# daniestevez/ldpc-toolbox

Hardware: AMD Instinct MI355X
Metric: codewords/s + info-bits/s, DVB-S2 n=64800 r=1/2 min-sum 50 iters (higher is better)
Workload: dtype f32

## Files before the change

ldpc_toolbox_amd/csrc/c_api.cpp:

```cpp
#include "../../include/ldpc_toolbox.h"

#include <algorithm>
#include <cerrno>
#include <cstdio>
#include <cstdlib>
#include <cstring>
#include <fstream>
#include <memory>
#include <sstream>
#include <string>
#include <vector>

#include "codes.h"
#include "demodulator.h"
#include "device_bch.h"
#include "device_decoder.h"
#include "device_encoder.h"
#include "device_nr_rm.h"
#include "device_nr_tb.h"
#include "encoder.h"
#include "implementation.h"
#include "simulator.h"
#include "sparse.h"

// ... 815 lines not shown
    *value = d.last_lanes();
  else if (k == "last_pooled")
    *value = static_cast<int64_t>(d.last_pooled());
  else if (k == "last_group")
    *value = static_cast<int64_t>(d.last_group());
  else if (k == "preferred_group")
    *value = static_cast<int64_t>(d.preferred_group(size_t(1) << 20));
  else if (k == "row_records")
    *value = d.row_records();
  else if (k == "record_flag_bits")
    *value = d.record_flag_bits();
  else if (k == "last_vn_records")
    *value = d.last_vn_records();
  else if (k == "last_vn_bundles")
    *value = d.last_vn_bundles();
  else if (k == "vn_bundle_saved_permille")
    *value = d.vn_bundle_saved_permille();
  else if (k == "last_vn_chains")
    *value = d.last_vn_chains();
  else if (k == "vn_chain_saved_permille")
    *value = d.vn_chain_saved_permille();
  else if (k == "flags8")
    *value = d.flags8();
  else if (k == "last_record_flag_bytes")
    *value = d.last_record_flag_bytes();
  else if (k == "call_edges")
    *value = d.call_edges();
  else if (k == "last_call_edges")
    *value = d.last_call_edges();
  else if (k == "minsum_correction")
    *value = static_cast<int64_t>(d.implementation().correction);
  else if (k == "minsum_correction_int")
    *value = d.implementation().correction_int;
  else if (k == "last_persist" || k == "experiments")
    *value = 0;
  else
    return -1;
  return 0;
}

int32_t ldpc_toolbox_decoder_set(void *decoder, const char *key, int64_t value) {
  auto *h = static_cast<DecoderHandle *>(decoder);
  if (!h || !h->dec || !key) return -1;
  const std::string k = key;
  if (k == "group_size" && value >= 0)
    h->dec->set_group_size(static_cast<size_t>(value));
// ... 574 lines not shown
```

ldpc_toolbox_amd/csrc/device_decoder.h:

```cpp
#pragma once
#include <hip/hip_runtime_api.h>

#include <algorithm>
#include <atomic>
#include <cstddef>
#include <cstdint>
#include <memory>
#include <string>
#include <vector>

#include "hip_owned.h"
#include "implementation.h"
#include "sparse.h"

namespace ldpc {

struct GroupCall;

struct KernelStat {
  uint64_t launches = 0;
  double total_ms = 0.0;
};

enum KernelKind { kKernelCheck = 0, kKernelVar = 1, kKernelLayer = 2, kKernelOther = 3, kKernelKinds = 4 };
// ... 5 lines not shown
  ~DeviceDecoder();

  size_t n() const { return n_; }
  size_t m() const { return m_; }
  size_t edges() const { return e_; }
  size_t input_len() const { return input_len_; }
  const Implementation &implementation() const { return impl_; }
  int device() const { return device_; }
  uint32_t max_check_degree() const { return max_row_weight_; }
  uint32_t max_variable_degree() const { return max_col_weight_; }
  size_t layers() const { return level_ptr_.empty() ? 0 : level_ptr_.size() - 1; }
  uint32_t last_lanes() const { return last_lanes_; }
  uint64_t last_pooled() const { return last_pooled_; }
  size_t last_group() const { return last_group_; }
  uint32_t row_records() const { return (rec_ready_ && records_wanted() && opt_lfree_ && !opt_staged_minsum_) ? rec_w_ : 0; }
  uint32_t record_flag_bits() const { return row_records() ? rec_flag_bits_ : 0; }
  uint32_t last_vn_records() const { return last_vn_records_.load(std::memory_order_relaxed) ? 1 : 0; }
  uint32_t flags8() const { return opt_flags8_ ? 1 : 0; }
  uint32_t last_record_flag_bytes() const { return last_record_flag_bytes_.load(std::memory_order_relaxed); }
  uint32_t last_vn_bundles() const { return last_vn_bundles_.load(std::memory_order_relaxed) ? 1 : 0; }
  uint32_t vn_bundle_saved_permille() const { return last_vn_bundle_saved_.load(std::memory_order_relaxed); }
  uint32_t last_vn_chains() const { return last_vn_chains_.load(std::memory_order_relaxed) ? 1 : 0; }
  uint32_t vn_chain_saved_permille() const { return last_vn_chain_saved_.load(std::memory_order_relaxed); }
  uint32_t call_edges() const { return opt_call_edges_ ? 1 : 0; }
  uint32_t last_call_edges() const { return last_call_edges_.load(std::memory_order_relaxed); }
  static constexpr uint32_t kCallEdgeIngest = 1;
  static constexpr uint32_t kCallEdgeClose = 2;
  static constexpr uint32_t kCallEdgeEmit = 4;
  static constexpr uint32_t kCallEdgeCheckpoint = 8;

  void set_group_size(size_t g) { group_pref_ = g; }
  size_t group_size() const { return group_pref_; }
  void set_min_group(size_t g) { min_group_ = g; }
  size_t preferred_group(size_t batch) const { return pick_group(batch); }
  bool set_option(const std::string &key, int64_t value);
  void set_profiling(bool on);
  KernelStat kernel_stat(int kind);
  void reset_kernel_stats();

  int decode_device(const void *llrs, bool llrs_f64, size_t batch, uint32_t max_iterations,
                    uint8_t *bits, size_t out_len, int32_t *iterations, void *posterior,
                    hipStream_t stream);

  int decode_host(const void *llrs, bool llrs_f64, size_t batch, uint32_t max_iterations,
                  uint8_t *bits, size_t out_len, int32_t *iterations, void *posterior);

// ... 57 lines not shown
  std::string error_;

  uint32_t n_keep_ = 0, n_free_ = 0;
  uint32_t post_rows_keep_ = 0;
  bool opt_rec_long_ = false;
  bool opt_rec_quiet_ = true;
  bool opt_vn_event_ = true;
  bool opt_vn_records_ = false;
  bool opt_flags8_ = false;
  bool opt_vn_bundles_ = false;
  static constexpr uint32_t kVnBundleW = kStreamBlock / 64;
  uint32_t vn_bundle_saved_[kVnBundleW + 1] = {};
  std::atomic<bool> last_vn_bundles_{false};
  std::atomic<uint32_t> last_vn_bundle_saved_{0};
  bool opt_vn_chains_ = false;
  uint32_t opt_vn_chain_len_ = 8;
  static constexpr uint32_t kVnChainLens[3] = {4, 8, 16};
  struct VnChainAt {
    uint32_t rs_at = 0, var_at = 0, ptr_at = 0, n_blocks = 0;
    uint32_t saved = 0, saved_alone = 0;
  } vn_chain_at_[3];
  std::atomic<bool> last_vn_chains_{false};
  std::atomic<uint32_t> last_vn_chain_saved_{0};
  bool opt_call_edges_ = true;
  std::atomic<uint32_t> last_call_edges_{0};
  std::atomic<uint32_t> last_record_flag_bytes_{0};
  std::atomic<bool> last_vn_records_{false};
  uint32_t rec_w_ = 0;
  uint32_t rec_flag_bits_ = 0;
  bool rec_ready_ = false, rec_prefers_ = false;
  uint32_t opt_records_ = 1;
  bool records_wanted() const { return opt_records_ >= 2 || (opt_records_ == 1 && rec_prefers_); }
  uint32_t opt_rec_run_ = 8;
  bool opt_compact_ = true;
  uint32_t opt_compact_first_ = 0, opt_compact_every_ = 0;
  uint32_t opt_serial_levels_ = 512;
  uint32_t opt_cn_reg_ = 1;
  uint32_t opt_hl_reg_ = 1;
  bool opt_lane_threads_ = true, opt_throttle_ = false;
  uint32_t opt_lead_ = 0;
  bool opt_lane_pace_ = true;
  bool opt_hl_records_ = true;
  std::vector<uint32_t> level_maxdeg_;
  std::vector<uint32_t> level_rec_ptr_;
  bool lfree_ready_ = false, opt_lfree_ = true;
  std::vector<uint32_t> level_ptr_;
// ... 56 lines not shown
```

ldpc_toolbox_amd/csrc/device_decoder.hip:

```cpp
#define LDPC_GROUP_KERNELS_TU 1
#include "codes.h"
#include "device_decoder_internal.h"

namespace ldpc {

static bool is_dvbs2_half_rate_normal(const SparseMatrix::Csr &g) {
  if (g.n_cols != 64800 || g.n_rows != 32400) return false;
  SparseMatrix ref;
  if (!codes::dvbs2("R1_2", &ref)) return false;
  const SparseMatrix::Csr r = ref.csr();
  if (r.n_edges != g.n_edges || r.row_ptr != g.row_ptr) return false;
  std::vector<uint32_t> a, b;
  for (uint32_t row = 0; row < g.n_rows; row++) {
    a.assign(g.edge_col.begin() + g.row_ptr[row], g.edge_col.begin() + g.row_ptr[row + 1]);
    b.assign(r.edge_col.begin() + r.row_ptr[row], r.edge_col.begin() + r.row_ptr[row + 1]);
    std::sort(a.begin(), a.end());
    std::sort(b.begin(), b.end());
    if (a != b) return false;
  }
  return true;
}

bool DeviceDecoder::fail(const std::string &msg, hipError_t e) {
  static std::mutex m;
// ... 71 lines not shown
    *dst = upload(v, &e);
    return e == hipSuccess;
  };
  g.edge_col.resize(g.edge_col.size() + kTablePad, 0);
  bool ok = up(g.row_ptr, &d->d_row_ptr_) && up(g.edge_col, &d->d_edge_col_) && up(g.col_ptr, &d->d_col_ptr_) &&
            up(g.col_edge, &d->d_col_edge_);
  const bool flooding_minsum = impl.schedule == Schedule::Flooding && impl.rule == Rule::Minsum && !impl.i8;
  if (ok && flooding_minsum) {
    const LfreeTables lf = build_lfree_tables(g);
    if (lf.ready) {
      d->n_keep_ = lf.n_keep;
      d->n_free_ = lf.n_free;
      d->post_rows_keep_ = lf.post_rows_keep;
      ok = up(lf.aux, &d->d_edge_aux_) && up(lf.keep_var, &d->d_keep_var_) && up(lf.keep_ptr, &d->d_keep_ptr_) &&
           up(lf.keep_edge, &d->d_keep_edge_) && up(lf.free_var, &d->d_free_var_) && up(lf.free_ptr, &d->d_free_ptr_) &&
           up(lf.free_edge, &d->d_free_edge_);
      d->lfree_ready_ = ok;
    }
    const RowRecordTables rr = d->lfree_ready_ ? build_row_record_tables(g, lf, impl.f64) : RowRecordTables();
    if (rr.ready) {
      d->rec_prefers_ = rr.rec_prefers;
      d->rec_w_ = rr.rec_w;
      d->rec_flag_bits_ = rr.flag_bits;
      ok = up(rr.keep_pos, &d->d_keep_pos_) && up(rr.peer, &d->d_edge_peer_) && up(rr.free_rs, &d->d_free_rs_);
      d->rec_ready_ = ok;
      const KeepRsTable kr = (ok && rr.flag_bits == 16) ? build_keep_rs(g, lf) : KeepRsTable();
      if (kr.ready) {
        const VnBundleTables vb = build_vn_bundles(lf.n_keep, lf.keep_ptr, lf.keep_var, kr.rs, kVnBundleW);
        std::vector<uint32_t> words = kr.rs;
        auto append = [&](const std::vector<uint32_t> &v) {
          const uint32_t at = static_cast<uint32_t>(words.size());
          words.insert(words.end(), v.begin(), v.end());
          return at;
        };
        d->bundle_rs_at_ = append(vb.keep_rs);
        d->bundle_var_at_ = append(vb.list_var);
        d->bundle_ptr_at_ = append(vb.list_ptr);
        for (uint32_t c = 0; c < 3; c++) {
          const VnChainTables vc = build_vn_chains(lf.n_keep, lf.keep_ptr, lf.keep_var, kr.rs, kVnBundleW, kVnChainLens[c]);
          VnChainAt &at = d->vn_chain_at_[c];
          at.rs_at = append(vc.keep_rs);
          at.var_at = append(vc.list_var);
          at.ptr_at = append(vc.list_ptr);
          at.n_blocks = vc.n_blocks;
          at.saved = vc.fetches ? static_cast<uint32_t>((vc.fetches - vc.issued) * 1000 / vc.fetches) : 0;
          at.saved_alone = vc.fetches ? static_cast<uint32_t>(vc.carried * 1000 / vc.fetches) : 0;
        }
        ok = up(words, &d->d_keep_rs_);
        for (uint32_t w = 2; w <= kVnBundleW; w++) {
          uint64_t fetches = 0, distinct = 0;
          count_vn_bundle_fetches(lf.n_keep, vb.list_ptr, vb.keep_rs, w, &fetches, &distinct);
          d->vn_bundle_saved_[w] = fetches ? static_cast<uint32_t>((fetches - distinct) * 1000 / fetches) : 0;
        }
      }
      d->opt_vn_records_ = kr.ready && ok && !impl.f64 && impl.correction == Correction::None && is_dvbs2_half_rate_normal(g);
      d->opt_flags8_ = d->opt_vn_records_;
      d->opt_vn_bundles_ = d->opt_vn_records_ && d->bundle_rs_at_ != 0;
      d->opt_vn_chains_ = d->opt_vn_bundles_ && d->vn_chain_at_[0].rs_at != 0;
    }
  }
  if (ok && flooding_minsum && !impl.f64) {
    SlicedTables st = build_sliced_tables(g);
    if (st.ready) {
      d->lat_ = std::make_unique<LatencyPath>();
      d->lat_->tables = std::move(st);
    }
  }
  if (ok && impl.schedule == Schedule::Flooding && impl.rule == Rule::Tanh && !impl.i8 && d->max_row_weight_ <= kLevelRecShort) {
    LevelTables all;
    all.level_ptr = {0u, g.n_rows};
    all.rows.resize(g.n_rows);
    for (uint32_t r = 0; r < g.n_rows; r++) all.rows[r] = r;
    all.maxdeg = {d->max_row_weight_};
    ok = up(build_level_recs(all, g.row_ptr, g.edge_col).words, &d->d_row_recs_);
  }
  LevelTables lt;
  if (ok && impl.schedule == Schedule::Layered) {
    lt = build_levels(g.row_ptr, g.edge_col, g.n_rows, g.n_cols);
    d->level_ptr_ = lt.level_ptr;
    d->level_maxdeg_ = lt.maxdeg;
    const LevelRecs lr = build_level_recs(lt, g.row_ptr, g.edge_col);
// ... 41 lines not shown
bool DeviceDecoder::set_option(const std::string &key, int64_t value) {
  if (value < 0) return false;
  const uint32_t v = static_cast<uint32_t>(value);
  if (key == "waves")
    opt_waves_ = v;
  else if (key == "vec")
    opt_vec_ = v;
  else if (key == "tile")
    opt_tile_ = v;
  else if (key == "lfree")
    opt_lfree_ = v != 0;
  else if (key == "records")
    opt_records_ = v != 0 ? (v >= 2 ? 2 : 1) : 0;
  else if (key == "rec_run")
    opt_rec_run_ = std::max<uint32_t>(v, 1);
  else if (key == "rec_quiet")
    opt_rec_quiet_ = v != 0;
  else if (key == "vn_event")
    opt_vn_event_ = v != 0;
  else if (key == "vn_records")
    opt_vn_records_ = v != 0;
  else if (key == "flags8")
    opt_flags8_ = v != 0;
  else if (key == "vn_bundles")
    opt_vn_bundles_ = v != 0;
  else if (key == "vn_chains")
    opt_vn_chains_ = v != 0;
  else if (key == "vn_chain_len") {
    if (v != kVnChainLens[0] && v != kVnChainLens[1] && v != kVnChainLens[2]) return false;
    opt_vn_chain_len_ = v;
  }
  else if (key == "rec_long")
    opt_rec_long_ = v != 0;
  else if (key == "call_edges")
    opt_call_edges_ = v != 0;
  else if (key == "compact")
    opt_compact_ = v != 0;
  else if (key == "staged_minsum")
    opt_staged_minsum_ = v != 0;
  else if (key == "hl_reg")
    opt_hl_reg_ = v;
  else if (key == "cn_reg")
    opt_cn_reg_ = v;
  else if (key == "hl_records")
    opt_hl_records_ = v != 0;
  else if (key == "lane_threads")
// ... 819 lines not shown
```

ldpc_toolbox_amd/csrc/graph_tables.h:

```cpp
#pragma once
#include <algorithm>
#include <cstdint>
#include <vector>

#include "record_flags8.h"
#include "slice_tasks.h"
#include "sparse.h"

namespace ldpc {

namespace dev {
enum : uint32_t { kAuxNone = 0xFFFFFFFFu, kAuxWriter = 0x80000000u, kAuxSingle = 0x7FFFFFFEu, kAuxMask = 0x7FFFFFFFu };
enum : uint32_t { kPeerKeep = 0x80000000u, kPeerPosMask = 0x7FFFFFFFu, kPeerWriter = 0x40000000u, kPeerRowMask = 0xFFFFFFu,
                  kPeerSingle = 0xFFFFFFu };
enum : uint32_t { kNoLane = 0xFFFFFFFFu };
}

constexpr uint32_t kTablePad = 16;

struct LfreeTables {
  bool ready = false;
  std::vector<uint32_t> aux, keep_var, keep_ptr{0}, keep_edge, free_var, free_ptr{0}, free_edge;
  uint32_t n_keep = 0, n_free = 0;
  uint32_t post_rows_keep = 0;
};
// ... 62 lines not shown
  }
  size_t far_peers = 0, near_peers = 0;
  for (size_t i = 0; i < lf.free_var.size(); i++) {
    const uint32_t v = lf.free_var[i], s0 = g.col_ptr[v], dv = g.col_ptr[v + 1] - s0;
    const uint32_t ea = g.col_edge[s0];
    t.free_rs[2 * i] = rs[ea];
    if (dv == 1) {
      t.peer[ea] = dev::kPeerWriter | (dev::kPeerSingle << 6);
      continue;
    }
    const uint32_t eb = g.col_edge[s0 + 1];
    t.peer[ea] = dev::kPeerWriter | rs[eb];
    t.peer[eb] = rs[ea];
    t.free_rs[2 * i + 1] = rs[eb];
    const uint32_t ra = rs[ea] >> 6, rb = rs[eb] >> 6;
    ((ra + 1 == rb || rb + 1 == ra) ? near_peers : far_peers) += 1;
  }
  t.rec_prefers = far_peers * 4 <= near_peers + far_peers;
  t.rec_w = g.max_row_weight <= rec_packed ? 3u : 4u;
  t.flag_bits = record_flag_bits(g.max_row_weight, f64);
  t.peer.resize(t.peer.size() + kTablePad, dev::kPeerKeep);
  t.ready = true;
  return t;
}

struct KeepRsTable {
  bool ready = false;
  std::vector<uint32_t> rs;
};
inline KeepRsTable build_keep_rs(const SparseMatrix::Csr &g, const LfreeTables &lf) {
  KeepRsTable t;
  if (!lf.ready || g.max_row_weight > 64 || g.n_rows >= dev::kPeerSingle) return t;
  std::vector<uint32_t> rs(std::max<uint32_t>(g.n_edges, 1));
  for (uint32_t r = 0; r < g.n_rows; r++)
    for (uint32_t e = g.row_ptr[r]; e < g.row_ptr[r + 1]; e++) rs[e] = (r << 6) | (e - g.row_ptr[r]);
  t.rs.reserve(lf.keep_edge.size() + kTablePad);
  for (uint32_t e : lf.keep_edge) t.rs.push_back(rs[e]);
  t.rs.resize(t.rs.size() + kTablePad, 0);
  t.ready = true;
  return t;
}

struct VnBundleTables {
  std::vector<uint32_t> list_var, list_ptr{0}, keep_rs;
  uint64_t fetches = 0, distinct = 0;
};
// ... 397 lines not shown
```

ldpc_toolbox_amd/csrc/kernels_flooding.hip.h:

```cpp
#pragma once
namespace ldpc {
namespace dev {



template <typename T>
struct RecWord {
  typedef uint32_t type;
  static constexpr int kArgShift = 26;
};
template <>
struct RecWord<double> {
  typedef uint64_t type;
  static constexpr int kArgShift = 58;
};

typedef uint32_t store_u32x4 __attribute__((ext_vector_type(4)));
__device__ __forceinline__ void store_data_pad(const store_u32x4 &data) { asm volatile("s_nop 0" ::"v"(data)); }

template <typename T, int VEC, bool NT>
__device__ __forceinline__ Pack<T, VEC> buf_load(const RowBuf &b, uint32_t lane_off, uint32_t row_off) {
  constexpr int kBytes = sizeof(T) * VEC;
  static_assert(kBytes == 4 || kBytes == 8 || kBytes == 16, "pack size");
  if constexpr (kBytes == 4)
// ... 950 lines not shown
        min1[k] = minsum_corrected(min1[k], mc...);
        min2[k] = minsum_corrected(min2[k], mc...);
      }
    }
    const uint32_t d = e1 - e0;
    for (uint32_t slot = 0; slot < d; slot++) {
      Pack<T, VEC> o;
#pragma unroll
      for (int k = 0; k < VEC; k++) {
        const uint32_t neg = uint32_t(sgn[k] >> slot) & 1u;
        const T mag = (arg[k] == slot) ? min2[k] : min1[k];
        o.v[k] = (tot[k] ^ neg) ? -mag : mag;
      }
      store_msg<T, VEC, NT>(msg + size_t(e0 + slot) * G, o);
    }
  }
  if (!FIRST) {
#pragma unroll
    for (int k = 0; k < VEC; k++)
      if (odd_acc[k]) unsat_out[off + k] = 1u;
  }
}

template <typename T, int VEC, int RECW, bool F16, int U, bool FIRST, bool NT, bool STREAM = false, bool LONG = true, bool SEND = true,
          bool F8 = false, typename... MC>
__global__ __launch_bounds__(256) void cn_minsum_rec_kernel(
    Graph g, Sched sc, State st, const T *__restrict__ chan, T *__restrict__ post, typename RecRef<T, F16, F8>::in rec_in,
    typename RecRef<T, F16, F8>::out rec_out, T *__restrict__ msg, uint32_t *__restrict__ unsat_out, uint32_t run, MC... mc) {
  static_assert(!F8 || (F16 && !LONG), "byte flags: rows of at most 7 edges");
  static_assert(!F8 || U == int(kRecFlags8MaxRow), "byte flags: a row is one round of 7 loads");
  typedef std::conditional_t<F8, RowRec8Once<T, VEC>, RowRec<T, VEC, RECW, RecFlagWord<T, F16, F8>>> Rec;
  constexpr bool CORR = sizeof...(MC) != 0;
  static_assert(is_corr_pack<T, MC...>, "mc: nothing, or one MinsumCorr<T>");
  typedef typename RecWord<T>::type W;
  if (group_finished(st)) return;
  const TablePtr row_ptr = table_ptr(g.row_ptr);
  const TablePtr edge_col = table_ptr(g.edge_col);
  const TablePtr edge_peer = table_ptr(g.edge_peer);
  const uint32_t *__restrict__ done = st.done;
  const uint32_t n_rows = g.n_rows, waves_per_chunk = sc.waves_per_chunk, tile = sc.tile;
  const uint32_t lane = threadIdx.x & 63u;
  const uint32_t wave = uniform((blockIdx.x * blockDim.x + threadIdx.x) >> 6);
  uint32_t chunk, node0;
  wave_slot(sc, wave, &chunk, &node0);
  if (chunk >= sc.nchunks) return;
  const uint32_t b0 = chunk * (64 * VEC);
  if (b0 >= *st.n_slots) return;
  const size_t off = size_t(b0) + lane * VEC;
  bool live[VEC];
  bool any_live = false, all_live = true;
#pragma unroll
  for (int k = 0; k < VEC; k++) {
    live[k] = done[off + k] == 0;
// ... 15 lines not shown
  const uint32_t in_tile = in_tile_of(b0, sc) * uint32_t(sizeof(T));
  const RowBuf b_chan = row_buf(chan + tile_base(b0, g.n_cols, sc), uint64_t(g.n_cols) * row_bytes - in_tile);
  const RowBuf b_post = row_buf(post + tile_base(b0, g.n_cols, sc), uint64_t(g.n_cols) * row_bytes - in_tile);
  const RowBuf b_msg = row_buf(msg + tile_base(b0, g.n_edges, sc), uint64_t(g.n_edges) * row_bytes - in_tile);
  RecBuf<F16> b_rin, b_rout;
  if constexpr (F16) {
    b_rin = rec_buf<T, RECW>(rec_in, b0, g.n_rows, sc, row_bytes);
    b_rout = rec_buf<T, RECW>(rec_out, b0, g.n_rows, sc, row_bytes);
  } else {
    b_rin.b = row_buf(rec_in + tile_base(b0, g.n_rows * RECW, sc), uint64_t(g.n_rows) * RECW * row_bytes - in_tile);
    b_rout.b = row_buf(rec_out + tile_base(b0, g.n_rows * RECW, sc), uint64_t(g.n_rows) * RECW * row_bytes - in_tile);
  }
  const uint32_t rec_bytes = Rec::kRows * row_bytes;
  __shared__ Pack<T, VEC> carry_chan[2][256], carry_msg[2][256];
  static_assert(sizeof(Pack<T, VEC>) * 256 * 4 <= 16384, "the hand-off arrays: 16 KiB per workgroup at most");
  uint64_t odd_m[VEC];
#pragma unroll
  for (int k = 0; k < VEC; k++) odd_m[k] = 0;

  for (uint32_t r = node0; r * run < n_rows; r += waves_per_chunk) {
    const uint32_t lo = r * run, hi = min(lo + run, n_rows);
    const uint32_t dir = (r & 1u) ? 0xFFFFFFFFu : 1u;
    uint32_t c = (r & 1u) ? hi - 1 : lo;
    Rec recA, recB;
    uint32_t carry_slot = kAuxNone;
    uint32_t carry_var = kAuxNone;
    uint32_t e0 = row_ptr[c], e1 = row_ptr[c + 1], ne0 = 0, ne1 = 0;
    if (c + dir < n_rows) {
      ne0 = row_ptr[c + dir];
      ne1 = row_ptr[c + dir + 1];
    }
    uint32_t cols[U], peers[U];
#pragma unroll
    for (int u = 0; u < U; u++) {
      cols[u] = edge_col[e0 + u];
      peers[u] = edge_peer[e0 + u];
    }
    if (!FIRST) recA.load(b_rin, lane_off, c * rec_bytes, row_bytes);

    auto row_step = [&](Rec &own, Rec &nxt, uint32_t ph) {
      const uint32_t d = e1 - e0, cn = c + dir, cp = c - dir;
      if (!FIRST && cn < n_rows) nxt.load(b_rin, lane_off, cn * rec_bytes, row_bytes);
      Pack<T, VEC> lv[U];
#pragma unroll
      for (int u = 0; u < U; u++)
        if (uint32_t(u) < d && cols[u] != carry_var)
// ... 273 lines not shown
```

ldpc_toolbox_amd/csrc/latency_paths.hip:

```cpp
#include "device_decoder_internal.h"

namespace ldpc {

static std::mutex g_latency_mutex;

struct DeviceDecoder::SmallBatchCall {
  DeviceDecoder &d;
  SmallBatchStaging &st;
  const bool host_pointers;
  const size_t batch;
  const void *const llrs;
  uint8_t *const bits;
  int32_t *const iterations;
  void *const posterior;
  const size_t in_bytes, bits_bytes, post_bytes;
  const void *d_llrs;
  uint8_t *d_bits;
  int32_t *d_iters;
  void *d_post;
  uint32_t *o_err = nullptr;

  SmallBatchCall(DeviceDecoder &dec, SmallBatchStaging &staging, const void *llrs_, bool llrs_f64, bool host, size_t batch_,
                 uint8_t *bits_, size_t out_len, int32_t *iterations_, void *posterior_)
      : d(dec), st(staging), host_pointers(host), batch(batch_), llrs(llrs_), bits(bits_), iterations(iterations_),
        posterior(posterior_), in_bytes(batch_ * dec.input_len_ * (llrs_f64 ? 8 : 4)), bits_bytes(batch_ * out_len),
        post_bytes(batch_ * dec.n_ * (llrs_f64 ? 8 : 4)), d_llrs(llrs_), d_bits(bits_), d_iters(iterations_), d_post(posterior_) {
    d.last_lanes_ = 1;
    d.last_group_ = batch;
    d.last_vn_records_.store(false, std::memory_order_relaxed);
    d.last_vn_bundles_.store(false, std::memory_order_relaxed);
    d.last_vn_bundle_saved_.store(0, std::memory_order_relaxed);
    d.last_vn_chains_.store(false, std::memory_order_relaxed);
    d.last_vn_chain_saved_.store(0, std::memory_order_relaxed);
    d.last_record_flag_bytes_.store(0, std::memory_order_relaxed);
  }

  int retreat() {
    d.opt_latency_ = 0;
    d.opt_latency_edge_ = 0;
    return kLatencyRetry;
  }
  int size_grid(const void *kernel_f32, const void *kernel_f64) {
    if (st.grid != 0) return 0;
    int cus = 0, per_cu_f = 0, per_cu_d = 0;
    hipError_t e = hipDeviceGetAttribute(&cus, hipDeviceAttributeMultiprocessorCount, d.device_);
    if (e == hipSuccess) e = hipOccupancyMaxActiveBlocksPerMultiprocessor(&per_cu_f, kernel_f32, 1024, 0);
    if (e == hipSuccess) e = hipOccupancyMaxActiveBlocksPerMultiprocessor(&per_cu_d, kernel_f64, 1024, 0);
    const int resident = e == hipSuccess ? cus * std::min(per_cu_f, per_cu_d) : 0;
    if (resident < 8) return retreat();
    st.grid = static_cast<uint32_t>(std::min(resident, 256));
    return 0;
  }
  int stage(size_t granule) {
    const size_t iters_at = round_up(256 + bits_bytes, 256), post_at = round_up(iters_at + batch * sizeof(int32_t), 256);
    const size_t out_need = host_pointers ? post_at + (posterior ? post_bytes : 0) : 256;
    if (st.h_out.ensure(out_need, granule) != hipSuccess || (host_pointers && st.h_in.ensure(in_bytes, granule) != hipSuccess)) {
// ... 192 lines not shown
```

ldpc_toolbox_amd/csrc/launch.hip.h:

```cpp
#pragma once
#include "device_decoder_internal.h"

namespace ldpc {

template <typename T>
struct Launch {
  hipStream_t s;
  bool rec_long;
  bool fast;
  bool corr;
  dev::MinsumCorr<T> minsum_corr;

  template <typename F>
  auto with_corr(F &&launch) const {
    if (corr) return launch(minsum_corr);
    return launch();
  }
  template <typename F>
  auto minsum(uint32_t vec, bool first, F &&f) const {
    return with_vec<T>(vec, [&](auto V) {
      return with_bool(first, [&](auto FIRST) { return with_corr([&](auto... mc) { return f(V, FIRST, mc...); }); });
    });
  }
  template <typename F>
// ... 43 lines not shown
  struct Records {
    T *mag;
    void *flags;
    uint32_t recw;
    bool flags8 = false;
  };
  template <typename F>
  static void with_rec_form(const Records &r, F &&f) {
    if (r.recw == 3 && r.flags != nullptr && r.flags8) return f(int_c<3>{}, std::true_type{}, std::true_type{});
    if (r.recw == 3 && r.flags != nullptr) return f(int_c<3>{}, std::true_type{}, std::false_type{});
    if (r.recw == 3) return f(int_c<3>{}, std::false_type{}, std::false_type{});
    f(int_c<4>{}, std::false_type{}, std::false_type{});
  }
  template <bool CONST, bool F16, bool F8 = false>
  static auto rec_ref(const Records &r) {
    using TT = std::conditional_t<CONST, const T, T>;
    using FW = dev::RecFlagWord<T, F16, F8>;
    if constexpr (F16)
      return dev::RecPair<TT, FW>{r.mag, static_cast<FW *>(r.flags)};
    else
      return static_cast<TT *>(r.mag);
  }
  void cn_rec(bool first, uint32_t vec, const Tiling &t, const dev::Graph &g, const dev::State &st, const T *chan, T *post,
              const Records &in, const Records &out, T *msg, uint32_t *unsat, uint32_t run, bool send = true) const {
    minsum(vec, first, [&](auto V, auto FIRST, auto... mc) {
      with_rec_form(in, [&](auto W, auto F16, auto F8) {
        with_bool(rec_long, [&](auto long_rows) {
          constexpr bool kF8 = decltype(F8)::value && !decltype(long_rows)::value;
          constexpr int kU = kF8 ? int(kRecFlags8MaxRow) : 8;
          auto go_rec = [&](auto SEND) {
            dev::cn_minsum_rec_kernel<T, decltype(V)::value, decltype(W)::value, decltype(F16)::value, kU, decltype(FIRST)::value,
                                      true, false, decltype(long_rows)::value, decltype(SEND)::value, kF8, decltype(mc)...>
                <<<t.blocks, t.threads, 0, s>>>(g, t.sched, st, chan, post, rec_ref<true, decltype(F16)::value, kF8>(in),
                                                rec_ref<false, decltype(F16)::value, kF8>(out), msg, unsat, run, mc...);
          };
          if constexpr (decltype(F16)::value) {
            if (!send) return go_rec(std::false_type{});
          }
          go_rec(std::true_type{});
        });
      });
    });
  }
  void vn_free_rec(uint32_t vec, const Tiling &t, const dev::Graph &g, const dev::State &st, const uint32_t *free_rs,
                   const T *chan, const Records &rec, T *post, int32_t event_iteration) const {
    with_vec<T>(vec, [&](auto V) {
      with_rec_form(rec, [&](auto W, auto F16, auto F8) {
        dev::vn_free_rec_kernel<T, decltype(V)::value, decltype(W)::value, decltype(F16)::value, decltype(F8)::value>
            <<<t.blocks, t.threads, 0, s>>>(g, t.sched, st, free_rs, chan, rec_ref<true, decltype(F16)::value, decltype(F8)::value>(rec),
                                            post, event_iteration);
      });
    });
  }
  void vn_free_hard(uint32_t vec, const Tiling &t, const dev::Graph &g, const dev::State &st, const uint32_t *free_rs,
                    const T *chan, const Records &rec, const T *post, uint64_t *bits, uint32_t W) const {
    with_vec<T>(vec, [&](auto V) {
      with_rec_form(rec, [&](auto RW, auto F16, auto F8) {
        dev::vn_free_hard_kernel<T, decltype(V)::value, decltype(RW)::value, decltype(F16)::value, decltype(F8)::value>
            <<<t.blocks, t.threads, 0, s>>>(g, t.sched, st, free_rs, chan, rec_ref<true, decltype(F16)::value, decltype(F8)::value>(rec),
                                            post, bits, W);
      });
    });
// ... 179 lines not shown
```

ldpc_toolbox_amd/csrc/run_group.hip.h:

```cpp
#pragma once
#include "launch.hip.h"

namespace ldpc {


template <typename T>
int DeviceDecoder::run_group(Workspace &w, const GroupCall &call) {
  const uint32_t max_iterations = call.max_iterations;
  const size_t nb = call.nb;
  uint32_t tile = opt_tile_ ? opt_tile_ : (sizeof(T) == 4 ? 256 : 128);
  tile = std::max<uint32_t>(64, tile / 64 * 64);
  while (w.G % tile != 0) tile -= 64;
  GroupFrame f(*this, w, call, tile);
  const uint32_t G = f.G, W = f.W, n = f.n, m = f.m;
  const hipStream_t s = f.s;
  const ProgressPoll &poll = f.poll;
  dev::State &st = f.st;
  auto ticked = [&](uint32_t it) { return f.ticked(it); };
  T *chan = static_cast<T *>(w.chan), *post = static_cast<T *>(w.post), *msg = static_cast<T *>(w.msg);
  const uint32_t target_waves = opt_waves_ ? opt_waves_ : 256 * 1024;
  const uint32_t lds_columns = impl_.rule == Rule::Tanh ? 1u : 2u;
  const Launch<T> launch{s, max_row_weight_ > 8 || opt_rec_long_, impl_.fast, impl_.correction != Correction::None,
                         dev::MinsumCorr<T>{static_cast<T>(impl_.alpha()), static_cast<T>(impl_.beta())}};
  const dev::Graph g = f.graph(d_edge_aux_.get<uint32_t>(), d_edge_peer_.get<uint32_t>());
// ... 77 lines not shown
    if (flags && flags8) {
      const dev::MoveList<uint8_t> fl{{reinterpret_cast<uint8_t *>(flags)}, {flag_rows}, {flag_rows}, 1};
      dev::compact_move_kernel<uint8_t><<<mv_t.blocks, mv_t.threads, 0, s>>>(w.plan, w.perm, w.slot_tmp, fl, tile,
                                                                           mv_t.sched.nchunks, mv_t.sched.waves_per_chunk);
    } else if (flags) {
      const dev::MoveList<uint16_t> fl{{flags}, {flag_rows}, {flag_rows}, 1};
      dev::compact_move_kernel<uint16_t><<<mv_t.blocks, mv_t.threads, 0, s>>>(w.plan, w.perm, w.slot_tmp, fl, tile,
                                                                            mv_t.sched.nchunks, mv_t.sched.waves_per_chunk);
    }
    grp::compact_commit(s, st, w.plan, w.unsat0, w.unsat1, w.n_slots, w.fill_cw, G);
  };
  auto checkpoint_due = [&](uint32_t it) {
    if (!opt_compact_ || max_iterations < 12 || it + 4 > max_iterations) return false;
    const bool layered = impl_.schedule == Schedule::Layered;
    const uint32_t first = opt_compact_first_ ? opt_compact_first_ : (layered ? 3u : 6u);
    const uint32_t every = opt_compact_every_ ? opt_compact_every_ : (layered ? 1u : 2u);
    if (it < first) return false;
    return it <= 26 ? (it - first) % every == 0 : it % 4 == 0;
  };

  uint32_t *unsat[2] = {w.unsat0, w.unsat1};
  int zero_fill = 0;
  last_record_flag_bytes_.store(0, std::memory_order_relaxed);

  if (impl_.schedule == Schedule::Flooding) {
    const bool streaming = fl_streaming;
    const uint32_t vec = pick_vec_for(tile, sizeof(T) == 4 ? 4 : 2, opt_vec_);
    const uint32_t stream_block = kStreamBlock;
    const Tiling vn_t = make_tiling(G, tile, 64 * vec, n, stream_block, opt_waves_ ? opt_waves_ : kVnWaves);
    Tiling cn_t = make_tiling(G, tile, 64 * vec, m, stream_block, target_waves);
    uint32_t st_threads = 256;
    size_t st_lds = 0;
    T *cn_scratch = nullptr;
    if (!streaming) {
      if (staged_block(lds_columns, max_row_weight_, sizeof(T), &st_threads, &st_lds)) {
        cn_t = make_tiling(G, tile, 64, m, st_threads, target_waves);
      } else {
        st_threads = kScratchThreads;
        st_lds = 0;
        cn_t = make_tiling(G, tile, 64, m, st_threads, std::min(target_waves, kScratchWaves));
        if (int rc = ensure_row_scratch(w, scratch_bytes_for(cn_t, max_row_weight_, sizeof(T)))) return rc;
        cn_scratch = w.row_scratch.get<T>();
      }
    }
    const uint32_t cn_reg = (streaming || !opt_cn_reg_ || !d_row_recs_ || impl_.rule != Rule::Tanh || impl_.fast ||
                             uint64_t(std::max(e_, n_)) * tile * sizeof(T) >= (1ull << 32))
// ... 1 lines not shown
                                : (max_row_weight_ <= 10 ? 10u : (max_row_weight_ <= 12 ? 12u : 0u));
    const bool wide_mask = max_row_weight_ > 32;
    const bool records = fl_records;
    const bool lfree = streaming && lfree_ready_ && opt_lfree_ && (w.msg2 != nullptr || records);
    T *mbuf[2] = {msg, (lfree && !records) ? static_cast<T *>(w.msg2) : msg};
    const bool flags8 = records && w.rec_flags[0] != nullptr && opt_flags8_ && !launch.rec_long &&
                        record_flag_bytes(max_row_weight_, sizeof(T) == 8) == 1;
    if (records) last_record_flag_bytes_.store((flags8 ? 1u : (w.rec_flags[0] ? 2u : uint32_t(sizeof(T)))),
                                  std::memory_order_relaxed);
    const typename Launch<T>::Records rbuf[2] = {{static_cast<T *>(w.rec[0]), w.rec_flags[0], rec_w_, flags8},
                                                 {static_cast<T *>(w.rec[1]), w.rec_flags[1], rec_w_, flags8}};
    const uint32_t rec_rows = w.rec_flags[0] ? 2 * m : m * rec_w_;
    if (lfree && post_rows_keep_ > 0 && post_rows_keep_ <= n) post_move_rows = post_rows_keep_;
    const bool vn_records = records && w.rec_flags[0] != nullptr && d_keep_rs_ && opt_vn_records_;
    last_vn_records_.store(vn_records, std::memory_order_relaxed);
    bool vn_bundles = false;
    const bool quiet = records && opt_rec_quiet_;
    if (quiet) {
      st.slice_state = w.slice_state;
      HIP_TRY(hipMemsetAsync(w.slice_state, 0, size_t(G / 64) * sizeof(uint32_t), s));
    }
    const uint32_t rec_run = std::max<uint32_t>(1, std::min<uint32_t>(opt_rec_run_, m));
    const Tiling rec_t = make_tiling(G, tile, 64 * vec, (m + rec_run - 1) / rec_run, stream_block, target_waves);
    dev::Graph g_keep = g, g_free = g;
    Tiling vn_keep_t = vn_t, vn_free_t = vn_t, vn_event_t = vn_t;
    if (lfree) {
      g_keep.list_var = d_keep_var_.get<uint32_t>();
      g_keep.list_ptr = d_keep_ptr_.get<uint32_t>();
      g_keep.list_edge = records ? d_keep_pos_.get<uint32_t>() : d_keep_edge_.get<uint32_t>();
      g_keep.n_list = n_keep_;
      g_free.list_var = d_free_var_.get<uint32_t>();
      g_free.list_ptr = d_free_ptr_.get<uint32_t>();
      g_free.list_edge = d_free_edge_.get<uint32_t>();
      g_free.n_list = n_free_;
      const uint32_t wv = opt_waves_ ? opt_waves_ : kVnWaves;
      vn_keep_t = make_tiling(G, tile, 64 * vec, n_keep_, stream_block, wv);
      vn_keep_t.sched.reverse = 1u;
      vn_free_t = make_tiling(G, tile, 64 * vec, n_free_, stream_block, wv);
      vn_event_t = make_tiling(G, tile, 64 * vec, n_free_, stream_block, 16 * 1024);
    }
    dev::Graph g_bundle = g_keep;
    uint32_t bundle_saved = 0, chain_rs_at = 0;
    if (vn_records && opt_vn_bundles_ && bundle_rs_at_ != 0) {
      vn_bundles = true;
      g_bundle.list_var = d_keep_rs_.get<uint32_t>() + bundle_var_at_;
      g_bundle.list_ptr = d_keep_rs_.get<uint32_t>() + bundle_ptr_at_;
// ... 20 lines not shown
        chain_rs_at = at.rs_at;
        chain_saved = chain.mates == kVnBundleW ? at.saved : at.saved_alone;
      }
    }
    last_vn_chains_.store(vn_chains, std::memory_order_relaxed);
    last_vn_chain_saved_.store(chain_saved, std::memory_order_relaxed);
    const bool adaptive = opt_compact_ && poll.flag != nullptr && poll.throttle && !opt_compact_every_;
    bool seen_drop = false;
    auto tail_checkpoint = [&](uint32_t it) {
      const uint32_t first_ck = opt_compact_first_ ? opt_compact_first_ : 6u;
      return seen_drop && max_iterations >= 12 && it + 4 <= max_iterations && it >= first_ck;
    };
    for (uint32_t it = 1; it <= max_iterations; it++) {
      if (it > 1 && poll.finished(it)) break;
      if (adaptive && !seen_drop && poll.running(static_cast<uint32_t>(nb)) < nb) seen_drop = true;
      const bool first = it == 1;
      uint32_t *unsat_out = unsat[it & 1];
      T *m_out = mbuf[it & 1];
      const T *m_in = mbuf[(it + 1) & 1];
      const dev::State stp = ticked(it);
      timed_begin(kKernelCheck, s);
      if (records)
        launch.cn_rec(first, vec, rec_t, g, stp, chan, (first && ingest_no_post) ? chan : post, rbuf[(it + 1) & 1], rbuf[it & 1],
                      msg, unsat_out, rec_run, !vn_records);
      else if (lfree)
        launch.cn_lfree(first, vec, wide_mask, cn_t, g, stp, chan, post, m_in, m_out, unsat_out);
      else if (streaming)
        launch.cn_minsum(first, vec, wide_mask, cn_t, g, stp, first ? chan : post, msg, unsat_out);
      else
        launch.cn_staged(first, impl_.rule, cn_reg, d_row_recs_.get<uint32_t>(), cn_t, st_lds, cn_scratch, g, stp, first ? chan : post, msg,
                         unsat_out, max_row_weight_);
      timed_end(kKernelCheck, s);
      timed_begin(kKernelVar, s);
      if (vn_records) {
        const bool event = quiet && it > 1 && opt_vn_event_;
        launch.vn_rec(vec, vn_chains ? vn_chain_t : vn_keep_t, vn_bundles ? g_bundle : g_keep, st, chan, rbuf[it & 1],
                      d_keep_rs_.get<uint32_t>() + (vn_chains ? chain_rs_at : (vn_bundles ? bundle_rs_at_ : 0u)), post,
                      first ? nullptr : unsat_out, unsat[(it + 1) & 1], static_cast<int32_t>(it) - 1, d_free_var_.get<uint32_t>(),
                      d_free_rs_.get<uint32_t>(), event ? &rbuf[(it - 1) & 1] : nullptr, n_free_, vn_chains ? &chain : nullptr);
        if (quiet && it > 1 && !event)
          launch.vn_free_rec(vec, vn_event_t, g_free, st, d_free_rs_.get<uint32_t>(), chan, rbuf[(it - 1) & 1], post,
                             static_cast<int32_t>(it) - 1);
      } else if (quiet && it > 1 && opt_vn_event_) {
        launch.vn_event(vec, vn_keep_t, g_keep, st, chan, m_out, post, unsat_out, unsat[(it + 1) & 1],
                        static_cast<int32_t>(it) - 1, d_free_var_.get<uint32_t>(), d_free_rs_.get<uint32_t>(), rbuf[(it - 1) & 1],
                        n_free_);
      } else {
// ... 131 lines not shown
```

Baseline: 51600.

## Add specialized check-node path for runs of rows with a fixed PN/NP shape

Classifies each check row by the pattern of its non-kept edges and marks rows with five kept edges followed by a previous/next staircase pair. Consecutive conforming rows get a span table, appended after the peer table on the device. The record check-node kernel then runs a specialized, fully unrolled loop over those runs. It carries the shared staircase variable through LDS between adjacent rows instead of decoding it through the generic peer/carry logic. This adds a new kernel instantiation and more code and registers, and it only applies to the byte-flag f32 path after the first iteration.

```diff
diff --git a/ldpc_toolbox_amd/csrc/c_api.cpp b/ldpc_toolbox_amd/csrc/c_api.cpp
--- a/ldpc_toolbox_amd/csrc/c_api.cpp
+++ b/ldpc_toolbox_amd/csrc/c_api.cpp
@@ -861,6 +861,14 @@
     *value = d.vn_chain_saved_permille();
   else if (k == "flags8")
     *value = d.flags8();
+  else if (k == "cn_row_shape")
+    *value = d.cn_row_shape();
+  else if (k == "last_cn_row_shape")
+    *value = d.last_cn_row_shape();
+  else if (k == "cn_row_shape_runs")
+    *value = d.cn_row_shape_runs();
+  else if (k == "cn_row_shape_rows")
+    *value = d.cn_row_shape_rows();
   else if (k == "last_record_flag_bytes")
     *value = d.last_record_flag_bytes();
   else if (k == "call_edges")
diff --git a/ldpc_toolbox_amd/csrc/device_decoder.h b/ldpc_toolbox_amd/csrc/device_decoder.h
--- a/ldpc_toolbox_amd/csrc/device_decoder.h
+++ b/ldpc_toolbox_amd/csrc/device_decoder.h
@@ -51,6 +51,10 @@
   uint32_t vn_bundle_saved_permille() const { return last_vn_bundle_saved_.load(std::memory_order_relaxed); }
   uint32_t last_vn_chains() const { return last_vn_chains_.load(std::memory_order_relaxed) ? 1 : 0; }
   uint32_t vn_chain_saved_permille() const { return last_vn_chain_saved_.load(std::memory_order_relaxed); }
+  uint32_t cn_row_shape() const { return opt_cn_row_shape_ ? 1 : 0; }
+  uint32_t last_cn_row_shape() const { return last_cn_row_shape_.load(std::memory_order_relaxed) ? 1 : 0; }
+  uint32_t cn_row_shape_runs() const { return last_cn_row_shape() ? last_cn_shape_runs_.load(std::memory_order_relaxed) : 0; }
+  uint32_t cn_row_shape_rows() const { return last_cn_row_shape() ? last_cn_shape_rows_.load(std::memory_order_relaxed) : 0; }
   uint32_t call_edges() const { return opt_call_edges_ ? 1 : 0; }
   uint32_t last_call_edges() const { return last_call_edges_.load(std::memory_order_relaxed); }
   static constexpr uint32_t kCallEdgeIngest = 1;
@@ -154,6 +158,11 @@
   } vn_chain_at_[3];
   std::atomic<bool> last_vn_chains_{false};
   std::atomic<uint32_t> last_vn_chain_saved_{0};
+  bool opt_cn_row_shape_ = false;
+  std::vector<uint32_t> row_shape_span_;
+  uint32_t row_shape_kind_ = 0;
+  std::atomic<bool> last_cn_row_shape_{false};
+  std::atomic<uint32_t> last_cn_shape_runs_{0}, last_cn_shape_rows_{0};
   bool opt_call_edges_ = true;
   std::atomic<uint32_t> last_call_edges_{0};
   std::atomic<uint32_t> last_record_flag_bytes_{0};
diff --git a/ldpc_toolbox_amd/csrc/device_decoder.hip b/ldpc_toolbox_amd/csrc/device_decoder.hip
--- a/ldpc_toolbox_amd/csrc/device_decoder.hip
+++ b/ldpc_toolbox_amd/csrc/device_decoder.hip
@@ -117,7 +117,16 @@
       d->rec_prefers_ = rr.rec_prefers;
       d->rec_w_ = rr.rec_w;
       d->rec_flag_bits_ = rr.flag_bits;
-      ok = up(rr.keep_pos, &d->d_keep_pos_) && up(rr.peer, &d->d_edge_peer_) && up(rr.free_rs, &d->d_free_rs_);
+      std::vector<uint32_t> peer_words = rr.peer;
+      if (peer_words.size() == size_t(g.n_edges) + kTablePad) {
+        const RowShapeTables shapes = build_row_shapes(g, rr, false);
+        if (shapes.kind != kRowShapeNone) {
+          d->row_shape_kind_ = shapes.kind;
+          d->row_shape_span_ = shapes.span;
+          peer_words.insert(peer_words.end(), d->row_shape_span_.begin(), d->row_shape_span_.end());
+        }
+      }
+      ok = up(rr.keep_pos, &d->d_keep_pos_) && up(peer_words, &d->d_edge_peer_) && up(rr.free_rs, &d->d_free_rs_);
       d->rec_ready_ = ok;
       const KeepRsTable kr = (ok && rr.flag_bits == 16) ? build_keep_rs(g, lf) : KeepRsTable();
       if (kr.ready) {
@@ -152,6 +161,7 @@
       d->opt_flags8_ = d->opt_vn_records_;
       d->opt_vn_bundles_ = d->opt_vn_records_ && d->bundle_rs_at_ != 0;
       d->opt_vn_chains_ = d->opt_vn_bundles_ && d->vn_chain_at_[0].rs_at != 0;
+      d->opt_cn_row_shape_ = d->opt_flags8_ && !d->row_shape_span_.empty();
     }
   }
   if (ok && flooding_minsum && !impl.f64) {
@@ -239,6 +249,8 @@
     opt_vn_records_ = v != 0;
   else if (key == "flags8")
     opt_flags8_ = v != 0;
+  else if (key == "cn_row_shape")
+    opt_cn_row_shape_ = v != 0;
   else if (key == "vn_bundles")
     opt_vn_bundles_ = v != 0;
   else if (key == "vn_chains")
diff --git a/ldpc_toolbox_amd/csrc/graph_tables.h b/ldpc_toolbox_amd/csrc/graph_tables.h
--- a/ldpc_toolbox_amd/csrc/graph_tables.h
+++ b/ldpc_toolbox_amd/csrc/graph_tables.h
@@ -1,6 +1,8 @@
 #pragma once
 #include <algorithm>
 #include <cstdint>
+#include <string>
+#include <utility>
 #include <vector>
 
 #include "record_flags8.h"
@@ -109,6 +111,99 @@
   t.peer.resize(t.peer.size() + kTablePad, dev::kPeerKeep);
   t.ready = true;
   return t;
+}
+
+constexpr uint32_t kRowShapeKept = 5;
+enum : uint32_t { kRowShapeNone = 0, kRowShapePN = 1, kRowShapeNP = 2 };
+struct RowShapeTables {
+  std::vector<std::string> signature;
+  std::vector<std::pair<std::string, uint32_t>> histogram;
+  uint32_t kind = kRowShapeNone;
+  std::vector<uint8_t> fits;
+  std::vector<uint32_t> span;
+  uint32_t fitting_rows = 0;
+};
+inline RowShapeTables build_row_shapes(const SparseMatrix::Csr &g, const RowRecordTables &rr, bool with_signatures = true) {
+  RowShapeTables t;
+  if (!rr.ready) return t;
+  const uint32_t M = g.n_rows;
+  if (with_signatures) t.signature.resize(M);
+  t.span.assign(M, 0);
+  std::vector<uint8_t> fits_pn(M, 0), fits_np(M, 0);
+  uint32_t n_pn = 0, n_np = 0;
+  std::vector<uint32_t> seen;
+  std::string s;
+  for (uint32_t c = 0; c < M; c++) {
+    const uint32_t e0 = g.row_ptr[c], d = g.row_ptr[c + 1] - e0;
+    uint32_t k = 0;
+    while (k < d && (rr.peer[e0 + k] & dev::kPeerKeep)) k++;
+    s = std::to_string(k);
+    s.push_back(':');
+    seen.clear();
+    for (uint32_t u = k; u < d; u++) {
+      const uint32_t p = rr.peer[e0 + u], prow = (p >> 6) & dev::kPeerRowMask;
+      char ch;
+      if (p & dev::kPeerKeep)
+        ch = 'K';
+      else if (prow == dev::kPeerSingle)
+        ch = 'S';
+      else if (std::find(seen.begin(), seen.end(), prow) != seen.end())
+        ch = 'T';
+      else if (prow + 1 == c)
+        ch = 'P';
+      else if (prow == c + 1)
+        ch = 'N';
+      else
+        ch = 'F';
+      if (!(p & dev::kPeerKeep) && prow != dev::kPeerSingle) seen.push_back(prow);
+      s.push_back(ch);
+    }
+    if (k == kRowShapeKept && d == kRowShapeKept + 2) {
+      const bool pn = s.compare(s.size() - 2, 2, "PN") == 0, np = s.compare(s.size() - 2, 2, "NP") == 0;
+      if (pn || np) {
+        const uint32_t p_slot = pn ? kRowShapeKept : kRowShapeKept + 1, n_slot = pn ? kRowShapeKept + 1 : kRowShapeKept;
+        const uint32_t pp = rr.peer[e0 + p_slot], pn_word = rr.peer[e0 + n_slot];
+        const bool fit = (pp & 63u) == n_slot && (pn_word & 63u) == p_slot && !(pp & dev::kPeerWriter) && (pn_word & dev::kPeerWriter);
+        (pn ? fits_pn : fits_np)[c] = fit;
+        (pn ? n_pn : n_np) += fit;
+      }
+    }
+    if (with_signatures) t.signature[c] = s;
+  }
+  t.kind = (n_pn == 0 && n_np == 0) ? kRowShapeNone : (n_pn >= n_np ? kRowShapePN : kRowShapeNP);
+  t.fits = t.kind == kRowShapeNP ? std::move(fits_np) : std::move(fits_pn);
+  t.fitting_rows = t.kind == kRowShapeNP ? n_np : n_pn;
+  for (uint32_t c = M; c-- > 0;)
+    if (t.fits[c]) t.span[c] = std::min<uint32_t>(0xFFFFu, 1 + (c + 1 < M ? (t.span[c + 1] & 0xFFFFu) : 0u));
+  for (uint32_t c = 0; c < M; c++)
+    if (t.fits[c]) t.span[c] |= std::min<uint32_t>(0xFFFFu, 1 + (c > 0 ? (t.span[c - 1] >> 16) : 0u)) << 16;
+  if (!with_signatures) return t;
+  std::vector<std::string> sorted = t.signature;
+  std::sort(sorted.begin(), sorted.end());
+  for (size_t i = 0; i < sorted.size();) {
+    size_t j = i;
+    while (j < sorted.size() && sorted[j] == sorted[i]) j++;
+    t.histogram.emplace_back(sorted[i], static_cast<uint32_t>(j - i));
+    i = j;
+  }
+  std::stable_sort(t.histogram.begin(), t.histogram.end(), [](const auto &a, const auto &b) { return a.second > b.second; });
+  return t;
+}
+inline bool row_shape_run_conforms(const std::vector<uint32_t> &span, uint32_t n_rows, uint32_t run, uint32_t r) {
+  const uint64_t lo = uint64_t(r) * run;
+  if (run == 0 || lo >= n_rows) return false;
+  const uint32_t hi = static_cast<uint32_t>(std::min<uint64_t>(lo + run, n_rows)), len = hi - static_cast<uint32_t>(lo);
+  const uint32_t w = span[(r & 1u) ? hi - 1 : static_cast<uint32_t>(lo)];
+  return ((r & 1u) ? w >> 16 : w & 0xFFFFu) >= len;
+}
+inline void count_row_shape_runs(const std::vector<uint32_t> &span, uint32_t n_rows, uint32_t run, uint32_t *runs, uint32_t *rows) {
+  *runs = *rows = 0;
+  if (run == 0 || span.size() < n_rows) return;
+  for (uint32_t r = 0; uint64_t(r) * run < n_rows; r++)
+    if (row_shape_run_conforms(span, n_rows, run, r)) {
+      *runs += 1;
+      *rows += static_cast<uint32_t>(std::min<uint64_t>(uint64_t(r) * run + run, n_rows) - uint64_t(r) * run);
+    }
 }
 
 struct KeepRsTable {
diff --git a/ldpc_toolbox_amd/csrc/kernels_flooding.hip.h b/ldpc_toolbox_amd/csrc/kernels_flooding.hip.h
--- a/ldpc_toolbox_amd/csrc/kernels_flooding.hip.h
+++ b/ldpc_toolbox_amd/csrc/kernels_flooding.hip.h
@@ -996,13 +996,18 @@
   }
 }
 
+enum : int { kCnShapeNone = 0, kCnShapePN = 1, kCnShapeNP = 2 };
+static_assert(kCnShapePN == int(kRowShapePN) && kCnShapeNP == int(kRowShapeNP), "the kinds of graph_tables.h, build_row_shapes");
 template <typename T, int VEC, int RECW, bool F16, int U, bool FIRST, bool NT, bool STREAM = false, bool LONG = true, bool SEND = true,
-          bool F8 = false, typename... MC>
+          bool F8 = false, int SHAPE = kCnShapeNone, typename... MC>
 __global__ __launch_bounds__(256) void cn_minsum_rec_kernel(
     Graph g, Sched sc, State st, const T *__restrict__ chan, T *__restrict__ post, typename RecRef<T, F16, F8>::in rec_in,
     typename RecRef<T, F16, F8>::out rec_out, T *__restrict__ msg, uint32_t *__restrict__ unsat_out, uint32_t run, MC... mc) {
   static_assert(!F8 || (F16 && !LONG), "byte flags: rows of at most 7 edges");
   static_assert(!F8 || U == int(kRecFlags8MaxRow), "byte flags: a row is one round of 7 loads");
+  static_assert(SHAPE == kCnShapeNone || ((SHAPE == kCnShapePN || SHAPE == kCnShapeNP) && F8 && !SEND && !FIRST && !STREAM),
+                "row shapes: the byte form without per-edge messages, behind the first iteration");
+  static_assert(kRowShapeKept + 2 <= kRecFlags8MaxRow, "the dominant shape is a row of the byte form");
   typedef std::conditional_t<F8, RowRec8Once<T, VEC>, RowRec<T, VEC, RECW, RecFlagWord<T, F16, F8>>> Rec;
   constexpr bool CORR = sizeof...(MC) != 0;
   static_assert(is_corr_pack<T, MC...>, "mc: nothing, or one MinsumCorr<T>");
@@ -1064,6 +1069,132 @@
     const uint32_t lo = r * run, hi = min(lo + run, n_rows);
     const uint32_t dir = (r & 1u) ? 0xFFFFFFFFu : 1u;
     uint32_t c = (r & 1u) ? hi - 1 : lo;
+    if constexpr (SHAPE != kCnShapeNone) {
+      const uint32_t span = edge_peer[g.n_edges + kTablePad + c];
+      if (((r & 1u) ? span >> 16 : span & 0xFFFFu) >= hi - lo) {
+        auto shape_run = [&](auto UP) {
+          constexpr bool kUp = decltype(UP)::value;
+          constexpr uint32_t K = kRowShapeKept, D = K + 2;
+          constexpr uint32_t NEXT = SHAPE == kCnShapePN ? K + 1 : K, PREV = SHAPE == kCnShapePN ? K : K + 1;
+          constexpr uint32_t AHEAD = kUp ? NEXT : PREV, BEHIND = kUp ? PREV : NEXT;
+          constexpr uint32_t kSgnMask8 = (1u << kRecFlags8MaxRow) - 1;
+          uint32_t cc = c, e0 = row_ptr[cc], cols[D];
+#pragma unroll
+          for (uint32_t u = 0; u < D; u++) cols[u] = edge_col[e0 + u];
+          Rec recA, recB;
+          {
+            const uint32_t far_off = (kUp ? cc - 1 : cc + 1) * rec_bytes;
+            const Pack<T, VEC> far_min1 = buf_load<T, VEC, false>(b_rin.b, lane_off, far_off);
+            const Pack<T, VEC> far_min2 = buf_load<T, VEC, false>(b_rin.b, lane_off, far_off + row_bytes);
+            const Pack<uint8_t, VEC> far_fl =
+                flags_load<uint8_t, VEC, false>(b_rin.f, lane_off / uint32_t(sizeof(T)), far_off / uint32_t(2 * sizeof(T)));
+            const Pack<T, VEC> chan_behind = buf_load<T, VEC, false>(b_chan, lane_off, cols[BEHIND] * row_bytes);
+            recA.load(b_rin, lane_off, cc * rec_bytes, row_bytes);
+            Pack<T, VEC> l_behind;
+#pragma unroll
+            for (int k = 0; k < VEC; k++) {
+              const T m_far = __builtin_bit_cast(T, record_flags8_value<W>(__builtin_bit_cast(W, far_min1.v[k]),
+                                                                              __builtin_bit_cast(W, far_min2.v[k]), far_fl.v[k], AHEAD));
+              l_behind.v[k] = chan_behind.v[k] + (recA.value(BEHIND, k) + m_far);
+            }
+            carry_chan[1][threadIdx.x] = l_behind;
+          }
+          auto step = [&](Rec &own, Rec &nxt, uint32_t ph) {
+            const uint32_t cn = kUp ? cc + 1 : cc - 1;
+            nxt.load(b_rin, lane_off, cn * rec_bytes, row_bytes);
+            Pack<T, VEC> lv[D];
+#pragma unroll
+            for (uint32_t u = 0; u < K; u++) lv[u] = buf_load<T, VEC, false>(b_post, lane_off, cols[u] * row_bytes);
+            lv[AHEAD] = buf_load<T, VEC, false>(b_chan, lane_off, cols[AHEAD] * row_bytes);
+            lv[BEHIND] = carry_chan[ph ^ 1u][threadIdx.x];
+            const uint32_t ne0 = kUp ? e0 + D : e0 - min(e0, D);
+            const TablePtr next_col = edge_col + ne0;
+            uint32_t ncols[D];
+#pragma unroll
+            for (uint32_t u = 0; u < D; u++) ncols[u] = next_col[u];
+            T min1[VEC], min2[VEC];
+            uint32_t sa[VEC];
+            uint64_t par_m[VEC];
+#pragma unroll
+            for (int k = 0; k < VEC; k++) {
+              min1[k] = Limits<T>::inf();
+              min2[k] = Limits<T>::inf();
+              sa[k] = 0;
+              par_m[k] = 0;
+            }
+            Pack<T, VEC> lnew;
+#pragma unroll
+            for (uint32_t u = 0; u < D; u++) {
+              uint32_t always = 1;
+              asm volatile("" : "+s"(always));
+              if (always)
+#pragma unroll
+              for (int k = 0; k < VEC; k++) {
+                T l = lv[u].v[k];
+                const T m_own = own.value(u, k);
+                if (u == AHEAD) {
+                  l = l + (m_own + nxt.value(BEHIND, k));
+                  lv[u].v[k] = l;
+                }
+                if (u == NEXT) lnew.v[k] = l;
+                const T x = l - m_own;
+                const T a = m_abs(x);
+                if (x < T(0.0)) sa[k] |= 1u << u;
+                par_m[k] ^= __builtin_amdgcn_ballot_w64(l <= T(0.0));
+                const bool lt1 = a < min1[k], lt2 = a < min2[k];
+                min2[k] = lt1 ? min1[k] : (lt2 ? a : min2[k]);
+                min1[k] = lt1 ? a : min1[k];
+                sa[k] = lt1 ? ((sa[k] & kSgnMask8) | (u << kArgShift16)) : sa[k];
+              }
+              if (u == AHEAD) carry_chan[ph][threadIdx.x] = lv[u];
+            }
+            if (write_post) {
+              if (all_live) {
+                buf_store<T, VEC, false>(b_post, lane_off, cols[NEXT] * row_bytes, lnew);
+              } else {
+#pragma unroll
+                for (int k = 0; k < VEC; k++)
+                  if (live[k]) row_store<T, false>(b_post, lane_off, cols[NEXT] * row_bytes + k * uint32_t(sizeof(T)), lnew.v[k]);
+              }
+            }
+            typename Rec::New out;
+            if constexpr (CORR) {
+#pragma unroll
+              for (int k = 0; k < VEC; k++) {
+                asm("" : "+v"(min1[k]));
+                asm("" : "+v"(min2[k]));
+                min1[k] = minsum_corrected(min1[k], mc...);
+                min2[k] = minsum_corrected(min2[k], mc...);
+                asm("" : "+v"(min1[k]));
+                asm("" : "+v"(min2[k]));
+              }
+            }
+#pragma unroll
+            for (int k = 0; k < VEC; k++) {
+              const uint32_t tot = __popc(sa[k] & kSgnMask8) & 1u;
+              odd_m[k] |= par_m[k];
+              out.min1.v[k] = min1[k];
+              out.min2.v[k] = min2[k];
+              out.flip.v[k] = uint16_t(tot ? sa[k] ^ kSgnMask8 : sa[k]);
+            }
+            out.template store<NT>(b_rout, lane_off, cc * rec_bytes, row_bytes);
+            cc = cn;
+            e0 = ne0;
+#pragma unroll
+            for (uint32_t u = 0; u < D; u++) cols[u] = ncols[u];
+          };
+          for (uint32_t i = lo; i < hi; i += 2) {
+            step(recA, recB, 0);
+            if (i + 1 < hi) step(recB, recA, 1);
+          }
+        };
+        if (r & 1u)
+          shape_run(std::false_type{});
+        else
+          shape_run(std::true_type{});
+        continue;
+      }
+    }
     Rec recA, recB;
     uint32_t carry_slot = kAuxNone;
     uint32_t carry_var = kAuxNone;
diff --git a/ldpc_toolbox_amd/csrc/latency_paths.hip b/ldpc_toolbox_amd/csrc/latency_paths.hip
--- a/ldpc_toolbox_amd/csrc/latency_paths.hip
+++ b/ldpc_toolbox_amd/csrc/latency_paths.hip
@@ -32,6 +32,9 @@
     d.last_vn_bundle_saved_.store(0, std::memory_order_relaxed);
     d.last_vn_chains_.store(false, std::memory_order_relaxed);
     d.last_vn_chain_saved_.store(0, std::memory_order_relaxed);
+    d.last_cn_row_shape_.store(false, std::memory_order_relaxed);
+    d.last_cn_shape_runs_.store(0, std::memory_order_relaxed);
+    d.last_cn_shape_rows_.store(0, std::memory_order_relaxed);
     d.last_record_flag_bytes_.store(0, std::memory_order_relaxed);
   }
 
diff --git a/ldpc_toolbox_amd/csrc/launch.hip.h b/ldpc_toolbox_amd/csrc/launch.hip.h
--- a/ldpc_toolbox_amd/csrc/launch.hip.h
+++ b/ldpc_toolbox_amd/csrc/launch.hip.h
@@ -89,22 +89,28 @@
       return static_cast<TT *>(r.mag);
   }
   void cn_rec(bool first, uint32_t vec, const Tiling &t, const dev::Graph &g, const dev::State &st, const T *chan, T *post,
-              const Records &in, const Records &out, T *msg, uint32_t *unsat, uint32_t run, bool send = true) const {
+              const Records &in, const Records &out, T *msg, uint32_t *unsat, uint32_t run, bool send = true,
+              uint32_t shape = kRowShapeNone) const {
     minsum(vec, first, [&](auto V, auto FIRST, auto... mc) {
       with_rec_form(in, [&](auto W, auto F16, auto F8) {
         with_bool(rec_long, [&](auto long_rows) {
           constexpr bool kF8 = decltype(F8)::value && !decltype(long_rows)::value;
           constexpr int kU = kF8 ? int(kRecFlags8MaxRow) : 8;
-          auto go_rec = [&](auto SEND) {
+          auto go_rec = [&](auto SEND, auto SHAPE) {
             dev::cn_minsum_rec_kernel<T, decltype(V)::value, decltype(W)::value, decltype(F16)::value, kU, decltype(FIRST)::value,
-                                      true, false, decltype(long_rows)::value, decltype(SEND)::value, kF8, decltype(mc)...>
+                                      true, false, decltype(long_rows)::value, decltype(SEND)::value, kF8, decltype(SHAPE)::value,
+                                      decltype(mc)...>
                 <<<t.blocks, t.threads, 0, s>>>(g, t.sched, st, chan, post, rec_ref<true, decltype(F16)::value, kF8>(in),
                                                 rec_ref<false, decltype(F16)::value, kF8>(out), msg, unsat, run, mc...);
           };
           if constexpr (decltype(F16)::value) {
-            if (!send) return go_rec(std::false_type{});
+            if constexpr (kF8 && !decltype(FIRST)::value && sizeof(T) == 4) {
+              if (!send && shape == kRowShapePN) return go_rec(std::false_type{}, int_c<dev::kCnShapePN>{});
+              if (!send && shape == kRowShapeNP) return go_rec(std::false_type{}, int_c<dev::kCnShapeNP>{});
+            }
+            if (!send) return go_rec(std::false_type{}, int_c<dev::kCnShapeNone>{});
           }
-          go_rec(std::true_type{});
+          go_rec(std::true_type{}, int_c<dev::kCnShapeNone>{});
         });
       });
     });
diff --git a/ldpc_toolbox_amd/csrc/run_group.hip.h b/ldpc_toolbox_amd/csrc/run_group.hip.h
--- a/ldpc_toolbox_amd/csrc/run_group.hip.h
+++ b/ldpc_toolbox_amd/csrc/run_group.hip.h
@@ -123,6 +123,7 @@
   uint32_t *unsat[2] = {w.unsat0, w.unsat1};
   int zero_fill = 0;
   last_record_flag_bytes_.store(0, std::memory_order_relaxed);
+  last_cn_row_shape_.store(false, std::memory_order_relaxed);
 
   if (impl_.schedule == Schedule::Flooding) {
     const bool streaming = fl_streaming;
@@ -170,6 +171,13 @@
     }
     const uint32_t rec_run = std::max<uint32_t>(1, std::min<uint32_t>(opt_rec_run_, m));
     const Tiling rec_t = make_tiling(G, tile, 64 * vec, (m + rec_run - 1) / rec_run, stream_block, target_waves);
+    uint32_t shape_runs = 0, shape_rows = 0;
+    if (vn_records && flags8 && opt_cn_row_shape_ && sizeof(T) == 4 && row_shape_span_.size() == m)
+      count_row_shape_runs(row_shape_span_, m, rec_run, &shape_runs, &shape_rows);
+    const bool cn_shape = shape_runs != 0 && max_iterations > 1;
+    last_cn_row_shape_.store(cn_shape, std::memory_order_relaxed);
+    last_cn_shape_runs_.store(cn_shape ? shape_runs : 0, std::memory_order_relaxed);
+    last_cn_shape_rows_.store(cn_shape ? shape_rows : 0, std::memory_order_relaxed);
     dev::Graph g_keep = g, g_free = g;
     Tiling vn_keep_t = vn_t, vn_free_t = vn_t, vn_event_t = vn_t;
     if (lfree) {
@@ -236,7 +244,7 @@
       timed_begin(kKernelCheck, s);
       if (records)
         launch.cn_rec(first, vec, rec_t, g, stp, chan, (first && ingest_no_post) ? chan : post, rbuf[(it + 1) & 1], rbuf[it & 1],
-                      msg, unsat_out, rec_run, !vn_records);
+                      msg, unsat_out, rec_run, !vn_records, (cn_shape && !first) ? row_shape_kind_ : uint32_t(kRowShapeNone));
       else if (lfree)
         launch.cn_lfree(first, vec, wide_mask, cn_t, g, stp, chan, post, m_in, m_out, unsat_out);
       else if (streaming)
```

After: 52320, median of 6. 1.4% higher.
